# Elliotshui/ABRSimulator

Hardware: NVIDIA B200
Metric: chunk_steps_per_sec (higher is better)
Workload: dtype f64

## Files before the change

abrsimulator_b200/csrc/abr_step.cu:

```cuda
#include <type_traits>

#include "abr_common.cuh"

namespace abr {

namespace {

constexpr int kStepBlock = 256;
#ifndef ABR_STEP_PF_DIST
#define ABR_STEP_PF_DIST 2
#endif
constexpr long long kPrefetchMinBytes = 192ll << 20;
constexpr int kTile = 128;
constexpr int kTileBlocksPerSM = 7;
constexpr int kStepTiles = 8;
constexpr int kRolloutBlock = 64;
constexpr int kStatsBlock = 256;
constexpr int kStatsSessionsPerBlock = 1024;
constexpr int kWrapGuard = 1 << 20;
#ifndef ABR_ROLLOUT_UNROLL
#define ABR_ROLLOUT_UNROLL 1
#endif
constexpr int kRolloutUnroll = ABR_ROLLOUT_UNROLL;

// ... 485 lines not shown
    const int T = v.trace_len[t];
    const double I = v.trace_interval[t];
    const double* bw = v.trace_bw + (size_t)t * v.T_max;
    double* c_row = cum + (size_t)t * cum_stride(v.T_max);
    double c = 0.0, mincap = kInf;
    c_row[0] = 0.0;
#pragma unroll 8
    for (int j = 0; j < T; ++j) {
        const double c_next = dadd(c, dmul(dmul(bw[j], v.p.payload), I));
        c_row[j + 1] = c_next;
        mincap = fmin(mincap, dsub(c_next, c));
        c = c_next;
    }
    for (int j = T + 1; j < cum_stride(v.T_max); ++j) c_row[j] = kInf;
    const bool ok = c > 0.0 && c < kInf && mincap > 0.0;
    int M = idx_stride(v.T_max) > 0 ? idx_cells(T) : 0;
    double scale = 0.0;
    if (M > 0 && ok) {
        scale = ddiv((double)M, c);
        if (!(scale > 0.0) || !(scale < kInf)) M = 0;
    } else {
        M = 0;
    }
    if (idx_stride(v.T_max) > 0) {
        uint16_t* i_row = idx + (size_t)t * idx_stride(v.T_max);
        int j = 1;
        for (int b = 0; b <= M; ++b) {
            while (j <= T - 1 && (int)cell_of(c_row[j], scale, M) < b) ++j;
            i_row[b] = (uint16_t)(j - 1);
        }
        for (int b = M + 1; b < idx_stride(v.T_max); ++b) i_row[b] = (uint16_t)(T > 0 ? T - 1 : 0);
    }
    ok_out[t] = ok ? 1 : 0;
    TraceMeta m;
    m.I = I; m.P = c; m.scale = scale; m.T = T; m.M = M;
    meta[t] = m;
}

__device__ __forceinline__ void reset_seg_phase(const double I, const int T, const double off, int& seg_out,
                                                double& phi_out, int& n_bad) {
    const double x = ddiv(off, I);
    const double n = floor(x);
    int seg = (n >= 0.0 && n < 2147483648.0) ? (int)((uint32_t)n % (uint32_t)T) : (int)fmod(n, (double)T);
    double phi = dsub(x, n);
    if (seg < 0 || seg >= T) { ++n_bad; seg = 0; }
    if (!(phi >= 0.0 && phi < 1.0)) { ++n_bad; phi = 0.0; }
    seg_out = seg; phi_out = phi;
}

__device__ __forceinline__ RawState reset_position(const EnvView& v, int tr, const double off, int& n_bad) {
    RawState w;
    if (tr < 0 || tr >= v.n_traces) { ++n_bad; tr = 0; }
    const int T = v.trace_len[tr];
    const double I = v.trace_interval[tr];
    int seg;
    reset_seg_phase(I, T, off, seg, w.phi, n_bad);
    const double* c_row = v.trace_cum + (size_t)tr * cum_stride(v.T_max);
    const double c0 = __ldg(c_row + seg), c1 = __ldg(c_row + seg + 1);
    w.pos = dadd(c0, dmul(dsub(c1, c0), w.phi));
    w.tr = tr; w.seg = seg; w.chunk = 0; w.last_q = v.p.default_quality; w.buffer = 0.0;
    return w;
}

__global__ void __launch_bounds__(kStepBlock)
abr_reset_kernel(EnvView v, const int32_t* __restrict__ trace_id, const double* __restrict__ start_offset,
                 uint32_t* __restrict__ draw_counter) {
    const int i = blockIdx.x * blockDim.x + threadIdx.x;
    if (i >= v.n) return;
    if (i == 0 && draw_counter) *draw_counter = 0u;
    int n_bad = 0;
    const RawState w = reset_position(v, trace_id[i], start_offset ? start_offset[i] : 0.0, n_bad);
    if (n_bad) atomicAdd(v.errors, (unsigned long long)n_bad);
    v.trace_id[i] = w.tr; v.seg[i] = w.seg; v.phi[i] = w.phi; v.pos[i] = w.pos; v.buffer[i] = 0.0; v.chunk[i] = 0;
    v.last_q[i] = v.p.default_quality; v.done[i] = 0; v.hist_len[i] = 0; v.last_pred[i] = 0.0; v.err_len[i] = 0;
    v.t_now[i] = 0.0; v.play_time[i] = 0.0; v.started[i] = v.p.start_up_length <= 0.0 ? 1 : 0;
    v.play_id[i] = 0; v.play_len[i] = 0.0;
#pragma unroll
    for (int j = 0; j < ABR_NUM_ACC; ++j) v.acc[(size_t)j * v.cap + i] = 0.0;
}

__device__ __forceinline__ void bulk_g2s(void* smem_dst, const void* gmem_src, uint32_t bytes, uint32_t mbar) {
    const uint32_t dst = (uint32_t)__cvta_generic_to_shared(smem_dst);
    asm volatile("cp.async.bulk.shared::cluster.global.mbarrier::complete_tx::bytes [%0], [%1], %2, [%3];"
                 ::"r"(dst), "l"(gmem_src), "r"(bytes), "r"(mbar) : "memory");
}

__device__ __forceinline__ void mbar_wait(uint32_t mbar, uint32_t parity) {
    for (int spins = 0; spins < (1 << 20); ++spins) {
        uint32_t done;
        asm volatile("{\n\t.reg .pred p;\n\tmbarrier.try_wait.parity.shared::cta.b64 p, [%1], %2;\n\tselp.u32 %0, 1, 0, p;\n\t}"
                     : "=r"(done) : "r"(mbar), "r"(parity) : "memory");
        if (done) return;
    }
    __trap();
}

__device__ __forceinline__ uint32_t row_bytes_of(int T) { return (uint32_t)((T + 5) / 2) * 16u; }
__device__ __forceinline__ uint32_t idx_bytes_of(int M) { return (uint32_t)((M + 1 + 7) / 8) * 16u; }

__device__ __forceinline__ int policy_action(const EnvView& v, const StepPolicy& pol, const int i) {
    const int A = v.A;
    const float* __restrict__ row = pol.logits + (size_t)i * A;
    const bool sample = pol.draw != nullptr;
    const uint32_t draw = sample ? __ldg(pol.draw) : 0u;
    const unsigned long long g = (unsigned long long)(v.session_base + (v.perm ? __ldg(v.perm + i) : i));
    float best = __int_as_float(0xff800000);
    int arg = 0;
    for (int a0 = 0; a0 < A; a0 += 4) {
        uint4 r = make_uint4(0u, 0u, 0u, 0u);
        if (sample) r = philox4x32_10((uint32_t)g, (uint32_t)(g >> 32), draw, (uint32_t)(a0 >> 2), pol.seed_lo, pol.seed_hi);
        const uint32_t w[4] = {r.x, r.y, r.z, r.w};
#pragma unroll
        for (int k = 0; k < 4; ++k) {
            if (a0 + k < A) {
                float x = __ldg(row + a0 + k);
                if (sample) {
                    const float u = __fmul_rn(__fadd_rn((float)(w[k] >> 9), 0.5f), 1.1920928955078125e-07f);
                    x = __fsub_rn(x, logf(-logf(u)));
                }
                if (x > best) { best = x; arg = a0 + k; }
            }
        }
    }
    return arg;
}

__device__ __forceinline__ void load_live(const EnvView& v, Sess& s, const int i, const double* __restrict__ speed,
                                          const bool fresh) {
    if (fresh) { s.t_now = 0.0; s.play_time = 0.0; s.play_len = 0.0; s.play_id = 0; s.started = v.p.start_up_length <= 0.0; }
    else {
        s.t_now = v.t_now[i]; s.play_time = v.play_time[i]; s.started = v.started[i] != 0;
        s.play_id = v.play_id[i]; s.play_len = v.play_len[i];
    }
    s.speed = speed ? speed + i : nullptr;
    s.speed_stride = (size_t)v.n; s.V = v.V; s.bad_speed = false;
}

template <bool LIVE>
__device__ __forceinline__ void store_state(const EnvView& v, const Sess& s, const int i) {
    v.seg[i] = s.seg; v.chunk[i] = s.chunk; v.last_q[i] = s.last_q; v.phi[i] = s.phi; v.pos[i] = s.pos;
    v.buffer[i] = s.buffer;
    if (LIVE) {
        v.t_now[i] = s.t_now; v.play_time[i] = s.play_time; v.started[i] = s.started ? 1 : 0;
        v.play_id[i] = s.play_id; v.play_len[i] = s.play_len;
    }
}

template <bool FAST, bool NOOUT, bool LIVE, typename OT>
__device__ __forceinline__ void store_step(const StepOutputs<OT>& o, const uint32_t ix, const StepRes& r) {
    if (NOOUT) {
    } else if (FAST) {
        __stcs(o.delay + ix, (OT)r.delay); __stcs(o.sleep + ix, (OT)r.sleep); __stcs(o.buffer + ix, (OT)r.buffer);
        __stcs(o.rebuf + ix, (OT)r.rebuf); __stcs(o.reward + ix, (OT)r.reward);
        o.eov[ix] = r.eov ? 1 : 0;
    } else {
        if (o.delay) __stcs(o.delay + ix, (OT)r.delay);
        if (o.sleep) __stcs(o.sleep + ix, (OT)r.sleep);
        if (o.buffer) __stcs(o.buffer + ix, (OT)r.buffer);
        if (o.rebuf) __stcs(o.rebuf + ix, (OT)r.rebuf);
        if (o.reward) __stcs(o.reward + ix, (OT)r.reward);
        if (o.eov) o.eov[ix] = r.eov ? 1 : 0;
        if (LIVE && o.latency) __stcs(o.latency + ix, (OT)r.latency);
    }
}

enum WinMode { kWinZero, kWinRoll, kWinKeep };

__device__ __forceinline__ void write_obs_window(const EnvView& v, const StepPolicyWindow& pol, const int i, const int chunk,
                                                 const int last_q, const double buffer, const bool done, const WinMode mode,
                                                 const double thr, const double delay) {
    const int W = pol.window, A = v.A, V = v.V;
    ABR_CHECK(i >= 0 && i < v.n && W >= 1 && W <= 32 && chunk >= 0 && (chunk < V || (done && chunk == V)),
              "windowed observation column / window / chunk");
    const size_t n = (size_t)v.n;
    float* __restrict__ ob = pol.obs + i;
    const int k_prev = chunk > 0 ? chunk - 1 : 0;
    __stcs(ob, last_q < 0 ? 0.0f : (float)dmul(__ldg(v.util + (size_t)k_prev * A + last_q), pol.w_util));
    __stcs(ob + n, (float)dmul(buffer, pol.w_buffer));
    __stcs(ob + 2 * n, (float)ddiv((double)(V - chunk), (double)V));
    float* __restrict__ wt = ob + 3 * n;
    float* __restrict__ wd = ob + (size_t)(3 + W) * n;
    if (mode == kWinRoll) {
        for (int w0 = 0; w0 < W - 1; w0 += 8) {
            float xt[8], xd[8];
#pragma unroll
            for (int k = 0; k < 8; ++k)
                if (w0 + k < W - 1) {
                    xt[k] = __ldcs(wt + (size_t)(w0 + k + 1) * n);
                    xd[k] = __ldcs(wd + (size_t)(w0 + k + 1) * n);
                }
#pragma unroll
            for (int k = 0; k < 8; ++k)
                if (w0 + k < W - 1) {
                    __stcs(wt + (size_t)(w0 + k) * n, xt[k]);
                    __stcs(wd + (size_t)(w0 + k) * n, xd[k]);
                }
        }
        __stcs(wt + (size_t)(W - 1) * n, (float)dmul(thr, pol.w_thr));
        __stcs(wd + (size_t)(W - 1) * n, (float)dmul(delay, pol.w_delay));
    } else if (mode == kWinZero) {
        for (int w = 0; w < W; ++w) {
            __stcs(wt + (size_t)w * n, 0.0f);
            __stcs(wd + (size_t)w * n, 0.0f);
        }
    }
    float* __restrict__ os = ob + (size_t)(3 + 2 * W) * n;
    for (int a = 0; a < A; ++a)
        __stcs(os + (size_t)a * n, done ? 0.0f : (float)dmul(__ldg(v.sizes + (size_t)chunk * A + a), pol.w_size));
}

template <int POL> struct PolicyArg { using type = StepPolicy; };
template <> struct PolicyArg<2> { using type = StepPolicyWindow; };
template <int POL> using PolicyArgs = typename PolicyArg<POL>::type;

template <bool SMEM, bool FAST, bool LIVE, int POL, typename OT>
__device__ __forceinline__ void step_session(const EnvView& v, Sess& s, const int i, const int q, const Lookup& lk,
                                             const PolicyArgs<POL>& pol, const double* __restrict__ speed,
                                             OT* __restrict__ o_delay, OT* __restrict__ o_sleep, OT* __restrict__ o_buffer,
                                             OT* __restrict__ o_rebuf, OT* __restrict__ o_reward, uint8_t* __restrict__ o_eov,
                                             OT* __restrict__ o_latency, OT* __restrict__ o_thr, OT* __restrict__ o_next_sizes) {
    if (LIVE) load_live(v, s, i, speed, false);
    StepRes r;
    step_core<SMEM, FAST, LIVE>(v, s, q, lk, r, (!FAST && v.p.track_history) || o_thr != nullptr || (POL && pol.obs));
    if (r.walk_error || (LIVE && s.bad_speed)) atomicAdd(v.errors, 1ull);
    if (FAST) {
        store_state<false>(v, s, i);
        __stcs(o_delay + i, (OT)r.delay); __stcs(o_sleep + i, (OT)r.sleep); __stcs(o_buffer + i, (OT)r.buffer);
        __stcs(o_rebuf + i, (OT)r.rebuf); __stcs(o_reward + i, (OT)r.reward);
        o_eov[i] = r.eov ? 1 : 0;
    } else {
        if (!r.inert) {
            store_state<LIVE>(v, s, i);
            if (v.p.track_history) {
                const int prev_len = r.reset_mpc ? 0 : s.hist_len - 1;
                ABR_CHECK(prev_len >= 0, "history length");
                if (!r.reset_mpc) v.bw_hist[(size_t)(prev_len % v.K) * v.cap + i] = r.thr;
                v.hist_len[i] = s.hist_len;
            }
            if (r.reset_mpc) { v.last_pred[i] = 0.0; v.err_len[i] = 0; }
            if (s.done) v.done[i] = 1;
            if (v.p.track_acc) {
                double* a = v.acc + i;
                const size_t c = v.cap;
                a[0 * c] = dadd(a[0 * c], r.reward); a[1 * c] = dadd(a[1 * c], r.rebuf); a[2 * c] = dadd(a[2 * c], r.u);
                a[3 * c] = dadd(a[3 * c], r.smooth); a[4 * c] = dadd(a[4 * c], r.sleep);
                a[5 * c] = dadd(a[5 * c], r.delay);
                a[6 * c] = dadd(a[6 * c], 1.0);
                if (r.eov) a[7 * c] = dadd(a[7 * c], 1.0);
                if (LIVE) {
                    a[8 * c] = dadd(a[8 * c], r.startup); a[9 * c] = dadd(a[9 * c], r.area);
                    a[10 * c] = dadd(a[10 * c], r.played);
                }
            }
        }
        if (o_delay) __stcs(o_delay + i, (OT)r.delay);
        if (o_sleep) __stcs(o_sleep + i, (OT)r.sleep);
        if (o_buffer) __stcs(o_buffer + i, (OT)r.buffer);
        if (o_rebuf) __stcs(o_rebuf + i, (OT)r.rebuf);
        if (o_reward) __stcs(o_reward + i, (OT)r.reward);
        if (o_eov) o_eov[i] = r.eov ? 1 : 0;
    }
    if (POL) {
        if (pol.action_out) pol.action_out[i] = q;
        if (pol.reward_sum) pol.reward_sum[i] = dadd(pol.reward_sum[i], r.reward);
        if constexpr (POL == 2) {
            write_obs_window(v, pol, i, s.chunk, s.last_q, s.buffer, !FAST && s.done,
                             r.inert ? kWinKeep : (r.reset_mpc ? kWinZero : kWinRoll), r.thr, r.delay);
        } else if (pol.obs) {
            ABR_CHECK(i >= 0 && i < v.n && (s.chunk >= 0 && (s.chunk < v.V || s.done)), "observation column / next chunk");
            float* __restrict__ ob = pol.obs + i;
            const size_t n = (size_t)v.n;
            const int A = v.A;
            __stcs(ob, (float)dmul(r.buffer, pol.s_buffer));
            __stcs(ob + n, (float)dmul(r.thr, pol.s_thr));
            __stcs(ob + 2 * n, (float)dmul(r.delay, pol.s_delay));
            __stcs(ob + 3 * n, (float)ddiv((double)q, (double)A));
            for (int a = 0; a < A; ++a)
                __stcs(ob + (size_t)(4 + a) * n,
                       (float)((!FAST && s.done) ? 0.0 : dmul(__ldg(v.sizes + s.chunk * A + a), pol.s_size)));
        }
    }
    if (o_latency) __stcs(o_latency + i, (OT)r.latency);
    if (o_thr) __stcs(o_thr + i, (OT)r.thr);
    if (o_next_sizes) {
        const int A = v.A;
        for (int a = 0; a < A; ++a)
            o_next_sizes[(size_t)i * A + a] = (OT)((!FAST && s.done) ? 0.0 : __ldg(v.sizes + s.chunk * A + a));
    }
}

template <bool FAST, bool LIVE, int POL, typename OT>
__global__ void __launch_bounds__(kTile, (LIVE || POL) ? 4 : kTileBlocksPerSM)
abr_step_kernel(EnvView v, const int32_t* __restrict__ action, const double* __restrict__ speed,
                OT* __restrict__ o_delay, OT* __restrict__ o_sleep, OT* __restrict__ o_buffer, OT* __restrict__ o_rebuf,
                OT* __restrict__ o_reward, OT* __restrict__ o_latency, OT* __restrict__ o_next_sizes,
                uint8_t* __restrict__ o_eov, OT* __restrict__ o_thr, int smem_doubles, int tiles_per_block,
                const PolicyArgs<POL> pol) {
    extern __shared__ __align__(16) double2 s_row2[];
    __shared__ __align__(8) unsigned long long s_mbar;
    __shared__ Quad s_meta;
    const uint32_t mbar = (uint32_t)__cvta_generic_to_shared(&s_mbar);
    if (smem_doubles != 0) {
        if (threadIdx.x == 0) {
            asm volatile("mbarrier.init.shared::cta.b64 [%0], 1;" ::"r"(mbar));
            asm volatile("fence.mbarrier_init.release.cluster;" ::: "memory");
        }
        __syncthreads();
// ... 59 lines not shown
                                                         o_reward, o_eov, o_latency, o_thr, o_next_sizes);
            }
            continue;
        }
        if (tr_first == tr_last && tr_first != staged) {
            __syncthreads();
            if (threadIdx.x == 0) {
                const Quad m0 = ldg256(v.trace_meta + tr_first);
                s_meta = m0;
                const int T0 = __double2loint(m0.d), M0 = __double2hiint(m0.d);
                const uint32_t rb = row_bytes_of(T0), ib = idx_bytes_of(M0);
                asm volatile("mbarrier.arrive.expect_tx.shared::cta.b64 _, [%0], %1;" ::"r"(mbar), "r"(rb + ib) : "memory");
                bulk_g2s(s_row, v.trace_cum + (size_t)tr_first * cum_stride(v.T_max), rb, mbar);
                bulk_g2s(s_idx, v.trace_idx + (size_t)tr_first * idx_stride(v.T_max), ib, mbar);
            }
            mbar_wait(mbar, parity);
            parity ^= 1u;
            staged = tr_first;
        }
        if (valid) {
            if (tr == staged) {
                make_sess(v, i, w, s, s_meta);
                s.cum_s = (uint32_t)__cvta_generic_to_shared(s_row);
                s.idx_s = (uint32_t)__cvta_generic_to_shared(s_idx);
#ifdef ABR_CHECKED
                s.chk_cum_n = smem_doubles; s.chk_idx_n = idx_stride(v.T_max);
                ABR_CHECK(row_bytes_of(s.T) <= 8u * (uint32_t)smem_doubles && idx_bytes_of(s.M) <= 2u * (uint32_t)idx_stride(v.T_max),
                          "staged rows fit the shared-memory buffer");
#endif
                step_session<true, FAST, LIVE, POL, OT>(v, s, i, q_cur, lk, pol, speed, o_delay, o_sleep, o_buffer, o_rebuf,
                                                        o_reward, o_eov, o_latency, o_thr, o_next_sizes);
            } else {
                make_sess(v, i, w, s);
                step_session<false, FAST, LIVE, POL, OT>(v, s, i, q_cur, lk, pol, speed, o_delay, o_sleep, o_buffer, o_rebuf,
                                                         o_reward, o_eov, o_latency, o_thr, o_next_sizes);
            }
        }
    }
}

__device__ __forceinline__ double session_cost(const EnvView& v, const double rebuf, const double smooth,
                                               const double played, const double startup, const double area) {
    double c = dadd(dmul(v.p.rebuf_penalty, rebuf), dmul(v.p.smooth_penalty, smooth));
    if (v.p.live) {
        c = dadd(c, dmul(v.p.startup_penalty, startup));
        c = dadd(c, dmul(v.p.latency_penalty, played > 0.0 ? ddiv(area, dmul(v.p.latency_tick, played)) : 0.0));
    }
    return c;
}

constexpr int kStatsGroup = 32;
constexpr int kStatsLanes = 4 * ABR_NUM_ACC;

__device__ __forceinline__ unsigned count_done(unsigned* counter) {
    unsigned old;
    asm volatile("atom.add.acq_rel.gpu.global.u32 %0, [%1], 1;" : "=r"(old) : "l"(counter) : "memory");
    return old;
}

__device__ __forceinline__ void stats_group_sum(const double* __restrict__ partials, const int n_partials, const int g,
                                                double* __restrict__ group_partials, double (*sm)[ABR_NUM_ACC]) {
    const int t = threadIdx.x;
    if (t < kStatsLanes) {
        const int q = t / ABR_NUM_ACC, j = t - q * ABR_NUM_ACC;
        const int b0 = g * kStatsGroup + q * 8;
        double x[8];
#pragma unroll
        for (int k = 0; k < 8; ++k)
            x[k] = b0 + k < n_partials ? __ldcg(partials + (size_t)(b0 + k) * ABR_NUM_ACC + j) : 0.0;
        double s = x[0];
#pragma unroll
        for (int k = 1; k < 8; ++k) s = dadd(s, x[k]);
        sm[q][j] = s;
    }
    __syncthreads();
    if (t < ABR_NUM_ACC) group_partials[(size_t)g * ABR_NUM_ACC + t] = dadd(dadd(dadd(sm[0][t], sm[1][t]), sm[2][t]), sm[3][t]);
}

__device__ __forceinline__ void stats_final_sum(const double* __restrict__ group_partials, const int n_groups,
                                                double* __restrict__ out, double (*sm)[ABR_NUM_ACC]) {
    const int t = threadIdx.x;
    __syncthreads();
    if (t < kStatsLanes) {
        const int q = t / ABR_NUM_ACC, j = t - q * ABR_NUM_ACC;
        double s = 0.0;
        for (int g0 = q; g0 < n_groups; g0 += 32) {
            double x[8];
#pragma unroll
            for (int k = 0; k < 8; ++k)
                x[k] = g0 + 4 * k < n_groups ? __ldcg(group_partials + (size_t)(g0 + 4 * k) * ABR_NUM_ACC + j) : 0.0;
#pragma unroll
            for (int k = 0; k < 8; ++k) s = dadd(s, x[k]);
        }
        sm[q][j] = s;
    }
    __syncthreads();
    if (t < ABR_NUM_ACC) out[t] = dadd(dadd(dadd(sm[0][t], sm[1][t]), sm[2][t]), sm[3][t]);
}

__device__ __forceinline__ void stats_finish(const double* __restrict__ partials, const int n_partials, const int b,
                                             const StatsScratch sc, double* __restrict__ out,
                                             double (*sm)[ABR_NUM_ACC], int* s_flag) {
    const int g = b / kStatsGroup;
    const int n_groups = (n_partials + kStatsGroup - 1) / kStatsGroup;
    const int g_size = min(kStatsGroup, n_partials - g * kStatsGroup);
    ABR_CHECK(b >= 0 && b < n_partials && g_size >= 1 && blockDim.x >= kStatsLanes, "block partial / group of the statistics");
    __syncthreads();
    if (threadIdx.x == 0) *s_flag = count_done(sc.counters + 1 + g) == (unsigned)(g_size - 1) ? 1 : 0;
    __syncthreads();
    if (!*s_flag) return;
    stats_group_sum(partials, n_partials, g, sc.group_partials, sm);
    __syncthreads();
    if (threadIdx.x == 0) {
        sc.counters[1 + g] = 0u;
        *s_flag = count_done(sc.counters) == (unsigned)(n_groups - 1) ? 1 : 0;
    }
    __syncthreads();
    if (!*s_flag) return;
    stats_final_sum(sc.group_partials, n_groups, out, sm);
    if (threadIdx.x == 0) sc.counters[0] = 0u;
}

template <typename OT>
struct RolloutOut {
    StepOutputs<OT> traj;
    const double* __restrict__ speed;
    const int32_t* __restrict__ in_trace_id;
    const double* __restrict__ in_offset;
    double* __restrict__ out_cost;
    double* __restrict__ out_stats;
    StatsScratch scratch;
};

struct EpisodeSums {
    double rew = 0.0, reb = 0.0, u = 0.0, sm = 0.0, sl = 0.0, dl = 0.0, su = 0.0, lat = 0.0, pl = 0.0;
    int steps = 0, eps = 0;
    bool reset_mpc = false;
};

template <bool LIVE, bool COUNT>
__device__ __forceinline__ void add_step(EpisodeSums& a, const StepRes& r, const EnvView& v, const Sess& s, const int i,
                                         const bool hist) {
    a.rew = dadd(a.rew, r.reward); a.reb = dadd(a.reb, r.rebuf); a.u = dadd(a.u, r.u);
    a.sm = dadd(a.sm, r.smooth); a.sl = dadd(a.sl, r.sleep); a.dl = dadd(a.dl, r.delay);
    if (LIVE) { a.su = dadd(a.su, r.startup); a.lat = dadd(a.lat, r.area); a.pl = dadd(a.pl, r.played); }
    if (COUNT) {
        a.steps += 1;
        a.eps += r.eov ? 1 : 0;
        if (r.reset_mpc) a.reset_mpc = true;
        else if (hist) v.bw_hist[(size_t)((s.hist_len - 1) % v.K) * v.cap + i] = r.thr;
    }
}

template <int POLICY, bool SMEM, bool FAST, bool NOOUT, bool LIVE, bool UNI, typename OT>
__device__ __forceinline__ void rollout_session(const EnvView& v, Sess& s, const int i, const uint32_t seed_lo,
                                                const uint32_t seed_hi, const int steps, const uint32_t step_base,
                                                const int32_t* __restrict__ actions_in, const RolloutOut<OT>& o,
                                                double (&acc_new)[ABR_NUM_ACC], const bool fresh) {
    constexpr bool AHEAD = (POLICY == ABR_POLICY_FIXED || POLICY == ABR_POLICY_RANDOM) && !LIVE;
    const unsigned long long gsession = (unsigned long long)(v.session_base + (v.perm ? __ldg(v.perm + i) : i));
    EpisodeSums sum;
    const int chunk_in = s.chunk;
    bool flagged = false;
    const uint32_t n = (uint32_t)v.n;
    const bool hist = !FAST && v.p.track_history != 0;
    const bool prev_ladder = v.p.smooth_prev_ladder != 0;
    uint32_t packed = 0u;
    if (LIVE) load_live(v, s, i, o.speed, fresh);
    auto action_at = [&](const int t) -> int {
        if (POLICY == ABR_POLICY_FIXED) {
            int a = __ldg(actions_in + (size_t)(t < steps ? t : steps - 1) * n + i);
            if (a < 0 || a >= v.A) { flagged = true; a = a < 0 ? 0 : v.A - 1; }
            return a;
        }
        if (POLICY == ABR_POLICY_RANDOM) {
            const uint32_t tg = step_base + (uint32_t)t;
            if ((tg & 7u) == 0u || t == 0) {
                uint32_t k_lo = seed_lo, k_hi = seed_hi;
                asm volatile("" : "+r"(k_lo), "+r"(k_hi));
                const uint4 r = philox4x32_10((uint32_t)gsession, (uint32_t)(gsession >> 32), tg >> 3, 0u,
                                              k_lo, k_hi);
                const uint32_t A = (uint32_t)v.A;
                auto two = [A](uint32_t x) { return (((x & 0xffffu) * A) >> 16) | ((((x >> 16) * A) >> 16) << 4); };
                packed = two(r.x) | (two(r.y) << 8) | (two(r.z) << 16) | (two(r.w) << 24);
            }
            return (int)((packed >> (4 * (tg & 7u))) & 0xfu);
        }
        if (POLICY == ABR_POLICY_RATE || POLICY == ABR_POLICY_BOLA) {
            if (!FAST && s.done) return 0;
            const int row = s.chunk * v.A;
            ABR_CHECK(s.chunk >= 0 && s.chunk < v.V, "policy row");
            auto size_at = [&](const int a) -> double {
                return SMEM ? lds_f64(s.tab_s + 16u * (uint32_t)(row + a)) : __ldg(&s.tab[row + a].x);
            };
            if (POLICY == ABR_POLICY_RATE) return policy_rate(v, i, s.hist_len, size_at);
            return policy_bola(v, s.buffer, row, size_at);
        }
        return policy_bba(v, s.buffer);
    };
    const int V_ = v.V, dq_ = v.p.default_quality;
    const bool wraps = FAST || v.p.auto_reset;
    auto next_chunk = [&](const int chunk) -> int {
        const int c = chunk + 1;
        return (c >= V_ && wraps) ? 0 : c;
    };
    auto next_last_q = [&](const int chunk, const int q) -> int {
        return (chunk + 1 >= V_ && wraps) ? dq_ : q;
    };
    uint32_t ix = (uint32_t)i;
    StepRes r;
    LiveGate g;
    g.buffer = 0.0; g.rebuf = g.idle = 0.0;
    g.a.startup = g.a.area = g.a.played = g.a.tc = 0.0;
    const double inv_q = pow2_inverse(v.p.sleep_quantum);
    if (AHEAD) {
        const AbrParams& pl = v.p;
        const int Vr = v.V;
        int q0 = action_at(0);
        Lookup lk0 = lookup_tables<SMEM>(s, v.A, Vr, s.chunk, q0, s.last_q, prev_ladder);
        int c1 = next_chunk(s.chunk);
        int lq1 = next_last_q(s.chunk, q0);
        double u_dq = 0.0;
        if (UNI && dq_ >= 0) u_dq = SMEM ? lds_f64(s.tab_s + 16u * (uint32_t)dq_ + 8u) : __ldg(&s.tab[dq_].y);
        Head h;
        bool werr = false;
        head<SMEM>(s, dadd(s.pos, lk0.size), h, werr);
        const bool can_speculate = SMEM || s.M > 0;
        bool calm = true;
        const unsigned lanes = __activemask();
#pragma unroll kRolloutUnroll
        for (int t = 0; t < steps; ++t) {
            const int q1 = action_at(t + 1);
            Lookup lk1;
            if (UNI) {
                ABR_CHECK(c1 >= 0 && c1 < Vr && q1 >= 0 && c1 * v.A + q1 < s.chk_tab_n, "{size, utility} table entry");
                const double2 su = SMEM ? lds_f64x2(s.tab_s + 16u * (uint32_t)(c1 * v.A + q1)) : __ldg(s.tab + c1 * v.A + q1);
                lk1.size = su.x;
                lk1.u = su.y;
                lk1.u_prev = c1 != 0 ? lk0.u : (dq_ >= 0 ? u_dq : su.y);
            } else {
                lk1 = lookup_tables<SMEM>(s, v.A, Vr, c1, q1, lq1, prev_ladder);
            }
            Head h1;
            bool ok1 = false;
            if (calm && can_speculate) ok1 = head_fast<SMEM>(s, dadd(h.target, lk1.size), h1);
            ABR_CHECK((unsigned long long)ix < (unsigned long long)steps * n, "trajectory element index");
            const bool moved = step_tail<SMEM, FAST, false>(pl, Vr, s, h, q0, lk0, g, r, hist, inv_q);
            store_step<FAST, NOOUT, false>(o.traj, ix, r);
            if (!FAST && o.traj.actions) __stcs(o.traj.actions + ix, q0);
            if (FAST || !r.inert) add_step<false, !FAST>(sum, r, v, s, i, hist);
            calm = !__any_sync(lanes, moved);
            if (moved || !ok1) {
                const double raw = dadd(s.pos, lk1.size);
                if (!can_speculate || !head_fast<SMEM>(s, raw, h1)) head_any<SMEM>(s, raw, h1, werr);
            }
            h = h1;
            lk0 = lk1;
            q0 = q1;
            if (!UNI) lq1 = next_last_q(c1, q1);
            c1 = next_chunk(c1);
            ix += n;
        }
        flagged |= werr;
    } else {
        for (int t = 0; t < steps; ++t) {
            const int q = action_at(t);
            const Lookup lk = lookup_tables<SMEM>(s, v.A, v.V, s.chunk, q, s.last_q, prev_ladder);
            ABR_CHECK((unsigned long long)ix < (unsigned long long)steps * n, "trajectory element index");
            step_core<SMEM, FAST, LIVE>(v, s, q, lk, r, hist);
            flagged |= r.walk_error;
            store_step<FAST, NOOUT, LIVE>(o.traj, ix, r);
            if (!FAST && o.traj.actions) __stcs(o.traj.actions + ix, q);
            if (FAST || !r.inert) add_step<LIVE, true>(sum, r, v, s, i, hist);
            ix += n;
        }
    }
    if (FAST && AHEAD) {
        sum.steps = steps;
        sum.eps = (int)(((long long)chunk_in + steps) / v.V);
        sum.reset_mpc = sum.eps > 0;
    }
    if (flagged || (LIVE && s.bad_speed)) atomicAdd(v.errors, 1ull);
    store_state<LIVE>(v, s, i);
    if (hist) v.hist_len[i] = s.hist_len;
    if (sum.reset_mpc) { v.last_pred[i] = 0.0; v.err_len[i] = 0; }
    if (!FAST && s.done) v.done[i] = 1;
    if (fresh) {
        if (!hist) v.hist_len[i] = 0;
        if (!sum.reset_mpc) { v.last_pred[i] = 0.0; v.err_len[i] = 0; }
        if (FAST || !s.done) v.done[i] = 0;
        if (!LIVE) {
            v.t_now[i] = 0.0; v.play_time[i] = 0.0; v.started[i] = v.p.start_up_length <= 0.0 ? 1 : 0;
            v.play_id[i] = 0; v.play_len[i] = 0.0;
        }
    }
    double* a = v.acc + i;
    const size_t c = v.cap;
    const double add[ABR_NUM_ACC] = {sum.rew, sum.reb, sum.u, sum.sm, sum.sl, sum.dl,
                                     (double)sum.steps, (double)sum.eps,
                                     sum.su, sum.lat, sum.pl};
    double old[ABR_NUM_ACC];
#pragma unroll
    for (int j = 0; j < ABR_NUM_ACC; ++j) old[j] = fresh ? 0.0 : __ldcg(a + j * c);
#pragma unroll
    for (int j = 0; j < ABR_NUM_ACC; ++j) {
        acc_new[j] = dadd(old[j], add[j]);
        a[j * c] = acc_new[j];
    }
    if (o.out_cost) o.out_cost[i] = session_cost(v, acc_new[ABR_ACC_REBUF], acc_new[ABR_ACC_SMOOTH], acc_new[ABR_ACC_PLAY],
                                                 acc_new[ABR_ACC_STARTUP], acc_new[ABR_ACC_LATENCY]);
}

template <int POLICY, bool FAST, bool NOOUT, bool LIVE, bool UNI, typename OT>
#ifndef ABR_ROLLOUT_MINBLOCKS
#define ABR_ROLLOUT_MINBLOCKS 8
#endif
__global__ void __launch_bounds__(kRolloutBlock, LIVE ? 6 : ABR_ROLLOUT_MINBLOCKS)
abr_rollout_kernel(EnvView v, uint32_t seed_lo, uint32_t seed_hi, int steps, uint32_t step_base,
                   const int32_t* __restrict__ actions_in, RolloutOut<OT> o, int smem_doubles,
                   double* __restrict__ block_partials) {
    extern __shared__ __align__(16) double2 s_row2[];
    __shared__ __align__(8) unsigned long long s_mbar;
    __shared__ int s_tr0, s_staged;
    __shared__ double s_part[4][ABR_NUM_ACC];
    __shared__ int s_flag;
    asm volatile("griddepcontrol.launch_dependents;");
    const int i = blockIdx.x * blockDim.x + threadIdx.x;
    const bool valid = i < v.n;
    double acc_new[ABR_NUM_ACC];
#pragma unroll
    for (int j = 0; j < ABR_NUM_ACC; ++j) acc_new[j] = 0.0;
    Sess s;
    int tr = -1;
    const bool fresh = o.in_trace_id != nullptr;
    int n_bad = 0;
    double* s_row = reinterpret_cast<double*>(s_row2);
    uint16_t* s_idx = reinterpret_cast<uint16_t*>(s_row + smem_doubles);
    double2* s_tab = reinterpret_cast<double2*>(s_idx + idx_stride(v.T_max));
    const uint32_t mbar = (uint32_t)__cvta_generic_to_shared(&s_mbar);
    auto stage_rows = [&](const int tr0) {
        s_staged = 0;
        if (smem_doubles == 0 || tr0 < 0 || tr0 >= v.n_traces) return;
        asm volatile("mbarrier.init.shared::cta.b64 [%0], 1;" ::"r"(mbar));
        asm volatile("fence.mbarrier_init.release.cluster;" ::: "memory");
        const uint32_t rb = (uint32_t)cum_stride(v.T_max) * 8u, ib = (uint32_t)idx_stride(v.T_max) * 2u;
        const uint32_t tab_bytes = (uint32_t)(v.V * v.A) * 16u;
        asm volatile("mbarrier.arrive.expect_tx.shared::cta.b64 _, [%0], %1;" ::"r"(mbar), "r"(rb + ib + tab_bytes) : "memory");
        bulk_g2s(s_row, v.trace_cum + (size_t)tr0 * cum_stride(v.T_max), rb, mbar);
        bulk_g2s(s_idx, v.trace_idx + (size_t)tr0 * idx_stride(v.T_max), ib, mbar);
        bulk_g2s(s_tab, v.tab, tab_bytes, mbar);
        s_staged = 1;
    };
    if (valid) {
        if (fresh) {
            RawState w;
            w.tr = o.in_trace_id[i];
            if (threadIdx.x == 0) stage_rows(w.tr);
            const double off = o.in_offset ? o.in_offset[i] : 0.0;
            if (w.tr < 0 || w.tr >= v.n_traces) { ++n_bad; w.tr = 0; }
            w.seg = 0; w.chunk = 0; w.last_q = v.p.default_quality; w.phi = 0.0; w.pos = 0.0; w.buffer = 0.0;
            make_sess(v, i, w, s);
            reset_seg_phase(s.I, s.T, off, s.seg, s.phi, n_bad);
            s.done = false; s.hist_len = 0;
            tr = w.tr;
            v.trace_id[i] = tr;
            if (n_bad) atomicAdd(v.errors, (unsigned long long)n_bad);
        } else {
            tr = v.trace_id[i];
            if (threadIdx.x == 0) stage_rows(tr);
            load_sess(v, i, s);
        }
    }
    if (threadIdx.x == 0) s_tr0 = tr;
    __syncthreads();
    const int tr0 = s_tr0;
    const bool staged = s_staged != 0;
    const int same = __syncthreads_and((!valid || tr == tr0) ? 1 : 0);
    const bool use_smem = staged && same && __ldg(&v.trace_meta[tr0].M) > 0;
    if (staged) mbar_wait(mbar, 0u);
    if (use_smem) {
        if (valid) {
            s.cum_s = (uint32_t)__cvta_generic_to_shared(s_row);
            s.idx_s = (uint32_t)__cvta_generic_to_shared(s_idx);
            s.tab_s = (uint32_t)__cvta_generic_to_shared(s_tab);
            asm volatile("" : "+r"(s.cum_s), "+r"(s.tab_s), "+r"(s.idx_s));
#ifdef ABR_CHECKED
            s.chk_cum_n = smem_doubles; s.chk_idx_n = idx_stride(v.T_max);
            ABR_CHECK(cum_stride(v.T_max) <= smem_doubles && s.T + 4 < cum_stride(v.T_max), "staged rows fit the shared-memory buffer");
#endif
            if (fresh) s.pos = position_of<true>(s, s.seg, s.phi);
            rollout_session<POLICY, true, FAST, NOOUT, LIVE, UNI, OT>(v, s, i, seed_lo, seed_hi, steps, step_base, actions_in, o, acc_new, fresh);
        }
    } else if (valid) {
        if (fresh) s.pos = position_of<false>(s, s.seg, s.phi);
        rollout_session<POLICY, false, FAST, NOOUT, LIVE, UNI, OT>(v, s, i, seed_lo, seed_hi, steps, step_base, actions_in, o, acc_new, fresh);
    }
    if (block_partials) {
#pragma unroll
        for (int j = 0; j < ABR_NUM_ACC; ++j) {
            double x = acc_new[j];
#pragma unroll
            for (int d = 16; d > 0; d >>= 1) x = dadd(x, __shfl_down_sync(0xffffffffu, x, d));
            if ((threadIdx.x & 31) == 0) s_part[threadIdx.x >> 5][j] = x;
        }
        __syncthreads();
        if (threadIdx.x < ABR_NUM_ACC) {
            double x = s_part[0][threadIdx.x];
            for (int w = 1; w < kRolloutBlock / 32; ++w) x = dadd(x, s_part[w][threadIdx.x]);
            block_partials[(size_t)blockIdx.x * ABR_NUM_ACC + threadIdx.x] = x;
        }
        if (o.out_stats) {
            static_assert(kRolloutBlock >= kStatsLanes, "stats_finish needs 44 threads");
            stats_finish(block_partials, (int)gridDim.x, (int)blockIdx.x, o.scratch, o.out_stats, s_part, &s_flag);
        }
    }
}

__device__ __forceinline__ double block_sum(double x, double* sm) {
#pragma unroll
    for (int o = 16; o > 0; o >>= 1) x = dadd(x, __shfl_down_sync(0xffffffffu, x, o));
    const int w = threadIdx.x >> 5, l = threadIdx.x & 31;
    __syncthreads();
    if (l == 0) sm[w] = x;
    __syncthreads();
    if (w == 0) {
        x = (l < (int)(blockDim.x >> 5)) ? sm[l] : 0.0;
#pragma unroll
        for (int o = 16; o > 0; o >>= 1) x = dadd(x, __shfl_down_sync(0xffffffffu, x, o));
    }
    return x;
}

__global__ void __launch_bounds__(kStatsBlock)
abr_stats_stage1(EnvView v, double* __restrict__ partials) {
    __shared__ double sm[32];
    const int lo = blockIdx.x * kStatsSessionsPerBlock;
    const int hi = min(v.n, lo + kStatsSessionsPerBlock);
    double x[ABR_NUM_ACC];
#pragma unroll
    for (int j = 0; j < ABR_NUM_ACC; ++j) {
        x[j] = 0.0;
        for (int i = lo + threadIdx.x; i < hi; i += blockDim.x) x[j] = dadd(x[j], v.acc[(size_t)j * v.cap + i]);
    }
#pragma unroll
    for (int j = 0; j < ABR_NUM_ACC; ++j) {
        const double t = block_sum(x[j], sm);
        if (threadIdx.x == 0) partials[(size_t)blockIdx.x * ABR_NUM_ACC + j] = t;
    }
}

__global__ void __launch_bounds__(64)
abr_stats_stage2(const double* __restrict__ partials, int n_partials, StatsScratch sc, double* __restrict__ out) {
    __shared__ double sm[4][ABR_NUM_ACC];
    __shared__ int s_flag;
    asm volatile("griddepcontrol.wait;" ::: "memory");
    const int g = blockIdx.x;
    const int n_groups = (n_partials + kStatsGroup - 1) / kStatsGroup;
    stats_group_sum(partials, n_partials, g, sc.group_partials, sm);
    __syncthreads();
    if (threadIdx.x == 0) s_flag = count_done(sc.counters) == (unsigned)(n_groups - 1) ? 1 : 0;
    __syncthreads();
    if (!s_flag) return;
    stats_final_sum(sc.group_partials, n_groups, out, sm);
    if (threadIdx.x == 0) sc.counters[0] = 0u;
}

__global__ void __launch_bounds__(kStepBlock)
abr_qoe_cost_kernel(EnvView v, double* __restrict__ out) {
    const int i = blockIdx.x * blockDim.x + threadIdx.x;
    if (i >= v.n) return;
    const size_t c = v.cap;
    out[i] = session_cost(v, v.acc[ABR_ACC_REBUF * c + i], v.acc[ABR_ACC_SMOOTH * c + i], v.acc[ABR_ACC_PLAY * c + i],
                          v.acc[ABR_ACC_STARTUP * c + i], v.acc[ABR_ACC_LATENCY * c + i]);
}

template <int POLICY>
__global__ void __launch_bounds__(kStepBlock)
abr_policy_decide_kernel(EnvView v, int32_t* __restrict__ action) {
    const int i = blockIdx.x * blockDim.x + threadIdx.x;
    if (i >= v.n) return;
    const double b = v.buffer[i];
    int q;
    if (POLICY == ABR_POLICY_BBA) {
        q = policy_bba(v, b);
    } else if (!v.p.auto_reset && v.done[i]) {
        q = 0;
    } else {
        const int chunk = v.chunk[i];
        ABR_CHECK(chunk >= 0 && chunk < v.V, "policy row");
        const int row = chunk * v.A;
        auto size_at = [&](const int a) -> double { return __ldg(v.sizes + row + a); };
        q = POLICY == ABR_POLICY_RATE ? policy_rate(v, i, v.hist_len[i], size_at) : policy_bola(v, b, row, size_at);
    }
    action[i] = q;
}

constexpr int kLookaheadBlock = 128;
constexpr int kLookaheadMaxH = 8;

struct LookNode { double phi, pos, buffer, J; int seg; };

template <bool FAST>
__global__ void __launch_bounds__(kLookaheadBlock)
abr_lookahead_kernel(EnvView v, const int H, int32_t* __restrict__ action, double* __restrict__ best_value,
                     int32_t* __restrict__ best_seq) {
    __shared__ double s_val[kLookaheadBlock];
    __shared__ int s_leaf[kLookaheadBlock];
    __shared__ int s_err[kLookaheadBlock];
    const int A = v.A;
    const int per_warp = 32 / A;
    const int lane = threadIdx.x & 31;
    const int g = lane / A, a0 = lane - g * A;
    const int i = (int)((blockIdx.x * (kLookaheadBlock / 32) + (threadIdx.x >> 5)) * per_warp) + g;
    const bool active = g < per_warp && i < v.n;
    double best = 0.0;
    int best_leaf = 0, h = 0, n_leaves = 1;
    bool err = false;
    if (active) {
        Sess s;
        load_sess(v, i, s);
        h = s.done ? 0 : min(H, v.V - s.chunk);
        ABR_CHECK(h <= kLookaheadMaxH && s.chunk >= 0, "lookahead depth");
        for (int d = 1; d < h; ++d) n_leaves *= A;
        if (h > 0) {
            const bool prev_ladder = v.p.smooth_prev_ladder != 0;
            const int chunk0 = s.chunk, hist0 = s.hist_len;
            LookNode st[kLookaheadMaxH];
            int dig[kLookaheadMaxH];
            dig[0] = a0;
            for (int d = 1; d < h; ++d) dig[d] = 0;
            int k = 0, leaf = 0;
            double J = 0.0;
            for (;;) {
                for (int d = k; d < h; ++d) {
                    const int q = dig[d];
                    const Lookup lk = lookup_tables<false>(s, A, v.V, s.chunk, q, s.last_q, prev_ladder);
                    StepRes r;
                    step_core<false, FAST, false>(v, s, q, lk, r, false);
                    err |= r.walk_error;
                    J = dadd(J, r.reward);
                    if (d + 1 < h) {
                        LookNode& nd = st[d + 1];
                        nd.phi = s.phi; nd.pos = s.pos; nd.buffer = s.buffer; nd.J = J; nd.seg = s.seg;
                    }
                }
                if (leaf == 0 || J > best) { best = J; best_leaf = leaf; }
                int d = h - 1;
                while (d >= 1 && dig[d] == A - 1) dig[d--] = 0;
// ... 259 lines not shown
```

Baseline: 63.18 billion.

## Precompute random actions into shared-memory queue before trace staging wait

For the random policy, Philox-generated packed actions for up to seven 8-step blocks are computed per thread into a shared-memory column before waiting on the trace-staging mbarrier. The rollout loop then pops them, so RNG work overlaps the async copy instead of sitting inside the step loop. Loop-invariant parameters and output pointers are also pinned into registers with opaque prmt asm, and the eov store uses __stwb. This adds 7 KB of shared memory per block and register pressure, which may lower occupancy.

```diff
diff --git a/abrsimulator_b200/csrc/abr_step.cu b/abrsimulator_b200/csrc/abr_step.cu
--- a/abrsimulator_b200/csrc/abr_step.cu
+++ b/abrsimulator_b200/csrc/abr_step.cu
@@ -661,7 +661,7 @@
     } else if (FAST) {
         __stcs(o.delay + ix, (OT)r.delay); __stcs(o.sleep + ix, (OT)r.sleep); __stcs(o.buffer + ix, (OT)r.buffer);
         __stcs(o.rebuf + ix, (OT)r.rebuf); __stcs(o.reward + ix, (OT)r.reward);
-        o.eov[ix] = r.eov ? 1 : 0;
+        __stwb(o.eov + ix, (uint8_t)(r.eov ? 1 : 0));
     } else {
         if (o.delay) __stcs(o.delay + ix, (OT)r.delay);
         if (o.sleep) __stcs(o.sleep + ix, (OT)r.sleep);
@@ -1027,40 +1027,104 @@
     }
 }
 
+constexpr int kActWords = 7;
+constexpr uint32_t kActStride = 4u * kRolloutBlock;
+
+__device__ __forceinline__ void sts_u32(uint32_t addr, uint32_t x) {
+    asm volatile("st.shared.u32 [%0], %1;" ::"r"(addr), "r"(x) : "memory");
+}
+__device__ __forceinline__ uint32_t lds_u32(uint32_t addr) {
+    uint32_t x;
+    asm volatile("ld.shared.u32 %0, [%1];" : "=r"(x) : "r"(addr) : "memory");
+    return x;
+}
+
+__device__ __forceinline__ uint32_t in_reg(uint32_t x) { asm volatile("prmt.b32 %0, %0, 0, 0x3210;" : "+r"(x)); return x; }
+__device__ __forceinline__ int in_reg(int x) { return (int)in_reg((uint32_t)x); }
+__device__ __forceinline__ unsigned long long in_reg(unsigned long long x) {
+    return ((unsigned long long)in_reg((uint32_t)(x >> 32)) << 32) | in_reg((uint32_t)x);
+}
+__device__ __forceinline__ double in_reg(double x) {
+    return __longlong_as_double((long long)in_reg((unsigned long long)__double_as_longlong(x)));
+}
+template <typename T>
+__device__ __forceinline__ T* in_reg(T* p) { return reinterpret_cast<T*>(in_reg((unsigned long long)p)); }
+
+__device__ __forceinline__ unsigned long long session_key(const EnvView& v, const int i) {
+    return (unsigned long long)(v.session_base + (v.perm ? __ldg(v.perm + i) : i));
+}
+
+struct ActionQueue {
+    uint32_t col;
+    uint32_t slot;
+    uint32_t end;
+    uint32_t cur;
+
+    __device__ __forceinline__ void fill(const unsigned long long key, const uint32_t blk, const uint32_t last,
+                                         const uint32_t seed_lo, const uint32_t seed_hi, const uint32_t A) {
+        const uint32_t span = ((last >> 3) - blk) & 0x1fffffffu;
+        const int n_words = span < (uint32_t)kActWords ? (int)span + 1 : kActWords;
+        slot = col;
+        end = col + kActStride * (uint32_t)n_words;
+        uint32_t k_lo = seed_lo, k_hi = seed_hi;
+        asm volatile("" : "+r"(k_lo), "+r"(k_hi));
+#pragma unroll
+        for (int k = 0; k < kActWords; ++k) {
+            if (k < n_words) {
+                const uint4 r = philox4x32_10((uint32_t)key, (uint32_t)(key >> 32), (blk + k) & 0x1fffffffu, 0u,
+                                              k_lo, k_hi);
+                auto two = [A](uint32_t x) { return (((x & 0xffffu) * A) >> 16) | ((((x >> 16) * A) >> 16) << 4); };
+                sts_u32(col + kActStride * k, two(r.x) | (two(r.y) << 8) | (two(r.z) << 16) | (two(r.w) << 24));
+            }
+        }
+    }
+    __device__ __forceinline__ uint32_t pop() {
+        const uint32_t x = lds_u32(slot);
+        slot += kActStride;
+        return x;
+    }
+    __device__ __forceinline__ void start(uint32_t* column, const unsigned long long key, const uint32_t first,
+                                          const uint32_t last, const uint32_t seed_lo, const uint32_t seed_hi,
+                                          const uint32_t A) {
+        col = (uint32_t)__cvta_generic_to_shared(column);
+        fill(key, first >> 3, last, seed_lo, seed_hi, A);
+        cur = pop() >> (4u * (first & 7u));
+    }
+    __device__ __forceinline__ int next(const uint32_t u, const bool first, const EnvView& v, const int i,
+                                        const uint32_t last, const uint32_t seed_lo, const uint32_t seed_hi) {
+        if (!first && (u & 7u) == 0u) {
+            if (slot == end) fill(session_key(v, i), u >> 3, last, seed_lo, seed_hi, (uint32_t)v.A);
+            cur = pop();
+        }
+        const int a = (int)(cur & 0xfu);
+        cur >>= 4;
+        return a;
+    }
+};
+
 template <int POLICY, bool SMEM, bool FAST, bool NOOUT, bool LIVE, bool UNI, typename OT>
 __device__ __forceinline__ void rollout_session(const EnvView& v, Sess& s, const int i, const uint32_t seed_lo,
                                                 const uint32_t seed_hi, const int steps, const uint32_t step_base,
-                                                const int32_t* __restrict__ actions_in, const RolloutOut<OT>& o,
-                                                double (&acc_new)[ABR_NUM_ACC], const bool fresh) {
+                                                const int32_t* __restrict__ actions_in, ActionQueue& acts,
+                                                const RolloutOut<OT>& o, double (&acc_new)[ABR_NUM_ACC],
+                                                const bool fresh) {
     constexpr bool AHEAD = (POLICY == ABR_POLICY_FIXED || POLICY == ABR_POLICY_RANDOM) && !LIVE;
-    const unsigned long long gsession = (unsigned long long)(v.session_base + (v.perm ? __ldg(v.perm + i) : i));
     EpisodeSums sum;
     const int chunk_in = s.chunk;
     bool flagged = false;
     const uint32_t n = (uint32_t)v.n;
     const bool hist = !FAST && v.p.track_history != 0;
     const bool prev_ladder = v.p.smooth_prev_ladder != 0;
-    uint32_t packed = 0u;
     if (LIVE) load_live(v, s, i, o.speed, fresh);
+    const uint32_t sb = POLICY == ABR_POLICY_RANDOM ? in_reg(step_base) : step_base;
     auto action_at = [&](const int t) -> int {
         if (POLICY == ABR_POLICY_FIXED) {
             int a = __ldg(actions_in + (size_t)(t < steps ? t : steps - 1) * n + i);
             if (a < 0 || a >= v.A) { flagged = true; a = a < 0 ? 0 : v.A - 1; }
             return a;
         }
-        if (POLICY == ABR_POLICY_RANDOM) {
-            const uint32_t tg = step_base + (uint32_t)t;
-            if ((tg & 7u) == 0u || t == 0) {
-                uint32_t k_lo = seed_lo, k_hi = seed_hi;
-                asm volatile("" : "+r"(k_lo), "+r"(k_hi));
-                const uint4 r = philox4x32_10((uint32_t)gsession, (uint32_t)(gsession >> 32), tg >> 3, 0u,
-                                              k_lo, k_hi);
-                const uint32_t A = (uint32_t)v.A;
-                auto two = [A](uint32_t x) { return (((x & 0xffffu) * A) >> 16) | ((((x >> 16) * A) >> 16) << 4); };
-                packed = two(r.x) | (two(r.y) << 8) | (two(r.z) << 16) | (two(r.w) << 24);
-            }
-            return (int)((packed >> (4 * (tg & 7u))) & 0xfu);
-        }
+        if (POLICY == ABR_POLICY_RANDOM)
+            return acts.next(sb + (uint32_t)t, t == 0, v, i, sb + (uint32_t)steps, seed_lo, seed_hi);
         if (POLICY == ABR_POLICY_RATE || POLICY == ABR_POLICY_BOLA) {
             if (!FAST && s.done) return 0;
             const int row = s.chunk * v.A;
@@ -1089,8 +1153,17 @@
     g.a.startup = g.a.area = g.a.played = g.a.tc = 0.0;
     const double inv_q = pow2_inverse(v.p.sleep_quantum);
     if (AHEAD) {
-        const AbrParams& pl = v.p;
-        const int Vr = v.V;
+        auto keep = [](auto x) { if constexpr (SMEM) return in_reg(x); else return x; };
+        AbrParams pl = v.p;
+        pl.rtt = keep(pl.rtt); pl.chunk_length = keep(pl.chunk_length); pl.max_buffer = keep(pl.max_buffer);
+        StepOutputs<OT> traj = o.traj;
+        if (FAST && !NOOUT) {
+            traj.delay = keep(traj.delay); traj.sleep = keep(traj.sleep); traj.buffer = keep(traj.buffer);
+            traj.rebuf = keep(traj.rebuf); traj.reward = keep(traj.reward); traj.eov = keep(traj.eov);
+        }
+        const int Vr = keep(v.V), Ar = keep(v.A), steps_r = keep(steps);
+        const uint32_t n_r = keep(n);
+        const bool dq_set = keep(dq_) >= 0;
         int q0 = action_at(0);
         Lookup lk0 = lookup_tables<SMEM>(s, v.A, Vr, s.chunk, q0, s.last_q, prev_ladder);
         int c1 = next_chunk(s.chunk);
@@ -1104,25 +1177,25 @@
         bool calm = true;
         const unsigned lanes = __activemask();
 #pragma unroll kRolloutUnroll
-        for (int t = 0; t < steps; ++t) {
+        for (int t = 0; t < steps_r; ++t) {
             const int q1 = action_at(t + 1);
             Lookup lk1;
             if (UNI) {
-                ABR_CHECK(c1 >= 0 && c1 < Vr && q1 >= 0 && c1 * v.A + q1 < s.chk_tab_n, "{size, utility} table entry");
-                const double2 su = SMEM ? lds_f64x2(s.tab_s + 16u * (uint32_t)(c1 * v.A + q1)) : __ldg(s.tab + c1 * v.A + q1);
+                ABR_CHECK(c1 >= 0 && c1 < Vr && q1 >= 0 && c1 * Ar + q1 < s.chk_tab_n, "{size, utility} table entry");
+                const double2 su = SMEM ? lds_f64x2(s.tab_s + 16u * (uint32_t)(c1 * Ar + q1)) : __ldg(s.tab + c1 * Ar + q1);
                 lk1.size = su.x;
                 lk1.u = su.y;
-                lk1.u_prev = c1 != 0 ? lk0.u : (dq_ >= 0 ? u_dq : su.y);
+                lk1.u_prev = c1 != 0 ? lk0.u : (dq_set ? u_dq : su.y);
             } else {
-                lk1 = lookup_tables<SMEM>(s, v.A, Vr, c1, q1, lq1, prev_ladder);
+                lk1 = lookup_tables<SMEM>(s, Ar, Vr, c1, q1, lq1, prev_ladder);
             }
             Head h1;
             bool ok1 = false;
             if (calm && can_speculate) ok1 = head_fast<SMEM>(s, dadd(h.target, lk1.size), h1);
             ABR_CHECK((unsigned long long)ix < (unsigned long long)steps * n, "trajectory element index");
             const bool moved = step_tail<SMEM, FAST, false>(pl, Vr, s, h, q0, lk0, g, r, hist, inv_q);
-            store_step<FAST, NOOUT, false>(o.traj, ix, r);
-            if (!FAST && o.traj.actions) __stcs(o.traj.actions + ix, q0);
+            store_step<FAST, NOOUT, false>(traj, ix, r);
+            if (!FAST && traj.actions) __stcs(traj.actions + ix, q0);
             if (FAST || !r.inert) add_step<false, !FAST>(sum, r, v, s, i, hist);
             calm = !__any_sync(lanes, moved);
             if (moved || !ok1) {
@@ -1133,8 +1206,8 @@
             lk0 = lk1;
             q0 = q1;
             if (!UNI) lq1 = next_last_q(c1, q1);
-            c1 = next_chunk(c1);
-            ix += n;
+            c1 = (c1 + 1 >= Vr && wraps) ? 0 : c1 + 1;
+            ix += n_r;
         }
         flagged |= werr;
     } else {
@@ -1199,6 +1272,7 @@
     __shared__ int s_tr0, s_staged;
     __shared__ double s_part[4][ABR_NUM_ACC];
     __shared__ int s_flag;
+    __shared__ uint32_t s_acts[kActWords][kRolloutBlock];
     asm volatile("griddepcontrol.launch_dependents;");
     const int i = blockIdx.x * blockDim.x + threadIdx.x;
     const bool valid = i < v.n;
@@ -1252,6 +1326,10 @@
     const bool staged = s_staged != 0;
     const int same = __syncthreads_and((!valid || tr == tr0) ? 1 : 0);
     const bool use_smem = staged && same && __ldg(&v.trace_meta[tr0].M) > 0;
+    ActionQueue acts;
+    if (POLICY == ABR_POLICY_RANDOM && valid)
+        acts.start(&s_acts[0][threadIdx.x], session_key(v, i), step_base, step_base + (uint32_t)steps, seed_lo, seed_hi,
+                   (uint32_t)v.A);
     if (staged) mbar_wait(mbar, 0u);
     if (use_smem) {
         if (valid) {
@@ -1264,11 +1342,13 @@
             ABR_CHECK(cum_stride(v.T_max) <= smem_doubles && s.T + 4 < cum_stride(v.T_max), "staged rows fit the shared-memory buffer");
 #endif
             if (fresh) s.pos = position_of<true>(s, s.seg, s.phi);
-            rollout_session<POLICY, true, FAST, NOOUT, LIVE, UNI, OT>(v, s, i, seed_lo, seed_hi, steps, step_base, actions_in, o, acc_new, fresh);
+            rollout_session<POLICY, true, FAST, NOOUT, LIVE, UNI, OT>(v, s, i, seed_lo, seed_hi, steps, step_base, actions_in, acts, o,
+                                                                      acc_new, fresh);
         }
     } else if (valid) {
         if (fresh) s.pos = position_of<false>(s, s.seg, s.phi);
-        rollout_session<POLICY, false, FAST, NOOUT, LIVE, UNI, OT>(v, s, i, seed_lo, seed_hi, steps, step_base, actions_in, o, acc_new, fresh);
+        rollout_session<POLICY, false, FAST, NOOUT, LIVE, UNI, OT>(v, s, i, seed_lo, seed_hi, steps, step_base, actions_in, acts, o,
+                                                                   acc_new, fresh);
     }
     if (block_partials) {
 #pragma unroll
diff --git a/profiles/ab_rollout_summary.py b/profiles/ab_rollout_summary.py
--- /dev/null
+++ b/profiles/ab_rollout_summary.py
@@ -0,0 +1,57 @@
+import glob
+import json
+import os
+import re
+import statistics
+import sys
+
+D = sys.argv[1] if len(sys.argv) > 1 else "/tmp/abr_ab"
+OLD = sys.argv[2] if len(sys.argv) > 2 else "old"
+
+
+def stat(xs):
+    return dict(median=statistics.median(xs), spread=max(xs) - min(xs), runs=xs) if xs else None
+
+
+def tr(kind, b):
+    out = []
+    for f in sorted(glob.glob(f"{D}/{kind}_{b}_*.txt")):
+        m = re.search(r"median ([0-9.]+) us", open(f).read())
+        if m:
+            out.append(float(m.group(1)))
+    return out
+
+
+def bench(b):
+    rows = []
+    for f in sorted(glob.glob(f"{D}/bench_{b}_*.json")):
+        lines = [l for l in open(f).read().splitlines() if l.startswith("{")]
+        if lines:
+            rows.append(json.loads(lines[-1]))
+    pick = {
+        "headline_us_per_step": lambda d: 1e3 * d["ms_per_step"],
+        "bba_policy_kernel_us": lambda d: 1e3 * d["bba_policy"]["kernel_ms"],
+        "fp32_outputs_kernel_us": lambda d: 1e3 * d["fp32_outputs"]["kernel_ms"],
+        "sorted_by_trace_kernel_us": lambda d: 1e3 * d["fused_kernel_layouts"]["sorted_by_trace"]["kernel_ms"],
+    }
+    for k, v in (rows[0]["fused_kernel_layouts"].items() if rows else []):
+        if k != "sorted_by_trace" and isinstance(v, dict) and "kernel_ms" in v:
+            pick[f"{k}_kernel_us"] = (lambda k: lambda d: 1e3 * d["fused_kernel_layouts"][k]["kernel_ms"])(k)
+    res = {}
+    for name, f in pick.items():
+        try:
+            res[name] = stat([f(d) for d in rows])
+        except (KeyError, TypeError):
+            pass
+    res["parity_non_identical_values"] = [d["parity"]["non_identical_values"] for d in rows]
+    res["clocks"] = rows[0].get("clocks") if rows else None
+    return res
+
+
+card = open(f"{D}/card.csv").read().strip().splitlines() if os.path.exists(f"{D}/card.csv") else []
+out = dict(card=card)
+for b in (OLD, "new"):
+    out[b] = dict(time_rollout_steps48_us=stat(tr("tr48", b)), time_rollout_steps1_us=stat(tr("tr1", b)), bench=bench(b))
+if os.path.exists(f"{D}/dump_cmp.txt"):
+    out["dump_outputs"] = open(f"{D}/dump_cmp.txt").read().strip().splitlines()[0]
+print(json.dumps(out, indent=1))
```

After: 65.79 billion (median of 6 runs). 4.1% higher.
